# michaelnny/muzero

Measured on AMD Instinct MI355X. Metric: self-play MCTS sims/sec (env-steps/sec = value / sims_per_move), higher is better.
Workload: dtype f32

## Files before the change

### include/mzlearner.h

```cpp
#ifndef MZLEARNER_H
#define MZLEARNER_H

#include <stdint.h>

#ifdef __cplusplus
extern "C" {
#endif

#define MZL_OK 0
#define MZL_E_INVALID (-1)
#define MZL_E_HIP (-2)
#define MZL_E_STATE (-3)

#define MZL_NET_MLP 0
#define MZL_NET_BOARD 1
#define MZL_NET_ATARI 2

typedef struct {
    int32_t in_dim;
    int32_t num_actions;
    int32_t num_planes;
    int32_t hidden_dim;
    int32_t value_support_size;
    int32_t reward_support_size;
// ... 15 lines not shown
    const int64_t* d_index;
    const float* d_weights;
    float* d_loss;
    float* d_priorities;
    int32_t batch;
    int32_t state_is_int8;
    int32_t action_bytes;
} mzl_batch;

typedef struct mz_learner mz_learner;

const char* mzl_last_error(void);


int mzl_create(const mzl_config* cfg, int device_id, mz_learner** out);
int mzl_destroy(mz_learner* h);

int64_t mzl_num_params(const mz_learner* h);
int64_t mzl_grad_floats(const mz_learner* h);
int32_t mzl_num_tensors(const mz_learner* h);
int mzl_tensor_info(const mz_learner* h, int32_t i, const char** name, int64_t* offset, int32_t* rows, int32_t* cols);
int32_t mzl_num_buffers(const mz_learner* h);
int64_t mzl_num_running(const mz_learner* h);
int mzl_buffer_info(const mz_learner* h, int32_t i, const char** name, int64_t* offset, int32_t* count);
int mzl_bind_buffers(mz_learner* h, float* d_running, int64_t* d_num_batches);

int mzl_bind(mz_learner* h, float* d_params, float* d_grads, float* d_exp_avg, float* d_exp_avg_sq);
int mzl_commit(mz_learner* h, void* stream);

int mzl_grad(mz_learner* h, const mzl_batch* batch, void* stream);
// ... 26 lines not shown
```

### muzero_amd/csrc/learner.hip

```cpp
#include <hip/hip_runtime.h>

#include <cmath>
#include <cstdio>
#include <cstdlib>
#include <cstring>
#include <string>
#include <vector>

#include "../../include/mzlearner.h"
#include "mz_learn.h"
#include "mz_learn_conv_host.h"

using namespace mzl;

static thread_local std::string g_err;
static int fail(int code, const std::string& msg) {
    g_err = msg;
    return code;
}
void mzl_internal_set_error(const std::string& msg) { g_err = msg; }
#define HIPCHK(expr)                                                                                                                     \
    do {                                                                                                                                 \
        hipError_t _e = (expr);                                                                                                          \
        if (_e != hipSuccess)                                                                                                            \
// ... 21 lines not shown
    int lds_heads = 0;
    std::vector<void*> allocs;
    DwJob* d_jobs = nullptr;
    DwBig* d_big = nullptr;
    std::vector<DwBig> big;
    std::vector<DwJob> jobs;
    int jobs_tiles = -1;
    float* d_sq = nullptr;
    int sq_blocks = 0;
    int num_cus = 256;
    const void* checked_ptr[9] = {};
    int fast_max_tiles = 16, stage_fast_max_tiles = 256;
    int chain_min_tiles = 96, chain_max_tiles = 1 << 30;
    float *params = nullptr, *grads = nullptr, *m = nullptr, *v = nullptr;
    bool committed = false;
    int back_parts = 1;
    bool fast = false;
};

static int tiles16(int x) { return (x + 15) / 16; }

extern "C" const char* mzl_last_error(void) { return g_err.c_str(); }

template <typename T>
static hipError_t dalloc(mz_learner* h, T** p, size_t count) {
    void* q = nullptr;
    hipError_t e = hipMalloc(&q, count * sizeof(T) + 256);
    if (e != hipSuccess) return e;
    e = hipMemset(q, 0, count * sizeof(T) + 256);
    h->allocs.push_back(q);
// ... 208 lines not shown
        h->fast = n.p_t <= 4 * LW && n.in_t <= 6 && n.h_t + n.a_t <= 6 && n.h_t <= 4 && n.a_t <= 2 && n.sv_t <= 2 && n.sr_t <= 2 && n.h_t * 64 <= LT &&
                  ks_ok(n.h_t, n.p_t) && ks_ok(n.a_t, n.p_t) && ks_ok(n.sv_t, n.p_t) && ks_ok(n.sr_t, n.p_t) && !getenv("MZL_GENERIC");
    }
    {
        const bool ok = h->fast && n.p_t % DX_PARTS == 0 && n.p_t / DX_PARTS <= LW && n.h_t <= 4 && LW % n.h_t == 0 && (n.p_t / DX_PARTS) % (LW / n.h_t) == 0 &&
                        (n.p_t / DX_PARTS) / (LW / n.h_t) <= 4 && n.h_t * 64 <= LT && !getenv("MZL_NO_SLICE");
        h->back_parts = ok ? DX_PARTS : 1;
    }
    build_jobs(h);
    build_big_jobs(h);
    if (dalloc(h, &h->d_jobs, h->jobs.size()) != hipSuccess || dalloc(h, &h->d_big, h->big.size()) != hipSuccess) return cleanup(fail(MZL_E_HIP, "hipMalloc failed (jobs)"));
    hipError_t e = hipSuccess;
    const void* stage_kernels[] = {(const void*)&k_learn_repr<true>,   (const void*)&k_learn_repr<false>, (const void*)&k_learn_unroll<true>,
                                   (const void*)&k_learn_unroll<false>, (const void*)&k_learn_back<true>,  (const void*)&k_learn_back<false>,
                                   (const void*)&k_learn_back_sliced<true>, (const void*)&k_learn_fwd_sliced<true>,
                                   (const void*)&k_learn_unroll<false, 3>, (const void*)&k_learn_dyn_chain, (const void*)&k_learn_dyn_back_chain};
    for (const void* f : stage_kernels)
        if (e == hipSuccess) e = hipFuncSetAttribute(f, hipFuncAttributeMaxDynamicSharedMemorySize, 160 * 1024);
    if (e == hipSuccess) e = hipFuncSetAttribute(reinterpret_cast<const void*>(&k_learn_dw), hipFuncAttributeMaxDynamicSharedMemorySize, LW * 8 * 256 * 4);
    if (e != hipSuccess) return cleanup(fail(MZL_E_HIP, std::string("hipFuncSetAttribute: ") + hipGetErrorString(e)));
    e = hipDeviceSynchronize();
    if (e != hipSuccess) return cleanup(fail(MZL_E_HIP, std::string("hipDeviceSynchronize: ") + hipGetErrorString(e)));
    *out = h;
    return MZL_OK;
}

extern "C" int mzl_destroy(mz_learner* h) {
    if (!h) return MZL_OK;
    (void)hipSetDevice(h->device);
    (void)hipDeviceSynchronize();
    if (h->conv) mzlc_destroy(h->conv);
    for (void* p : h->allocs) (void)hipFree(p);
    delete h;
    return MZL_OK;
}

extern "C" void* mzl_debug_stamps(const mz_learner* h) { return h ? h->sv.stamps : nullptr; }

extern "C" int64_t mzl_num_params(const mz_learner* h) { return !h ? 0 : (h->conv ? mzlc_num_params(h->conv) : h->P.total); }
extern "C" int64_t mzl_grad_floats(const mz_learner* h) {
    return !h ? 0 : (h->conv ? mzlc_num_params(h->conv) : (int64_t)h->P.total * h->cfg.grad_slices);
}
extern "C" int32_t mzl_num_tensors(const mz_learner* h) { return !h ? 0 : (h->conv ? mzlc_num_tensors(h->conv) : 2 * NLAYER); }
extern "C" int32_t mzl_num_buffers(const mz_learner* h) { return (h && h->conv) ? mzlc_num_buffers(h->conv) : 0; }
extern "C" int64_t mzl_num_running(const mz_learner* h) { return (h && h->conv) ? mzlc_num_running(h->conv) : 0; }
extern "C" int mzl_buffer_info(const mz_learner* h, int32_t i, const char** name, int64_t* offset, int32_t* count) {
    if (!h || !h->conv || mzlc_buffer_info(h->conv, i, name, offset, count) != MZL_OK) return fail(MZL_E_INVALID, "buffer index out of range");
// ... 10 lines not shown
    return MZL_OK;
}

extern "C" int mzl_tensor_info(const mz_learner* h, int32_t i, const char** name, int64_t* offset, int32_t* rows, int32_t* cols) {
    if (h && h->conv) {
        if (mzlc_tensor_info(h->conv, i, name, offset, rows, cols) != MZL_OK) return fail(MZL_E_INVALID, "tensor index out of range");
        return MZL_OK;
    }
    if (!h || i < 0 || i >= 2 * NLAYER) return fail(MZL_E_INVALID, "tensor index out of range");
    const LTensor& t = h->P.t[i];
    if (name) *name = h->names[i].c_str();
    if (offset) *offset = t.off;
    if (rows) *rows = t.n;
    if (cols) *cols = t.k;
    return MZL_OK;
}

extern "C" int mzl_bind(mz_learner* h, float* d_params, float* d_grads, float* d_exp_avg, float* d_exp_avg_sq) {
    if (!h || !d_params || !d_grads || !d_exp_avg || !d_exp_avg_sq) return fail(MZL_E_INVALID, "null argument to mzl_bind");
    if (h->conv) return mzlc_bind(h->conv, d_params, d_grads, d_exp_avg, d_exp_avg_sq);
    h->params = d_params; h->grads = d_grads; h->m = d_exp_avg; h->v = d_exp_avg_sq;
    h->committed = false;
    h->jobs_tiles = -1;
    return MZL_OK;
}

static int launch_adam(mz_learner* h, const AdamArgs& a, hipStream_t st) {
    int maxcnt = 0;
    for (int i = 0; i < 2 * NLAYER; i++) {
        const LTensor& t = h->P.t[i];
// ... 40 lines not shown
        static const char* names[9] = {"d_state", "d_action", "d_pi_prob", "d_value", "d_reward", "d_index", "d_weights", "d_loss", "d_priorities"};
        for (int i = 0; i < 9; i++) {
            if (ptrs[i] == h->checked_ptr[i]) continue;
            hipPointerAttribute_t at{};
            const hipError_t e = hipPointerGetAttributes(&at, ptrs[i]);
            if (e != hipSuccess || at.type != hipMemoryTypeDevice || at.device != h->device) {
                (void)hipGetLastError();
                return fail(MZL_E_INVALID, std::string(names[i]) + " is not memory of the learner's GPU (the batch is read where the replay lives: keep it in HBM)");
            }
            h->checked_ptr[i] = ptrs[i];
        }
    }
    if (b->action_bytes == 1 && h->cfg.num_actions > 128) return fail(MZL_E_INVALID, "num_actions > 128 needs int16 actions");
    HIPCHK(hipSetDevice(h->device));
    hipStream_t st = reinterpret_cast<hipStream_t>(stream);
    const LNet& n = h->net;
    LBatch bt{};
    bt.state = b->d_state; bt.action = b->d_action; bt.pi = b->d_pi_prob; bt.value = b->d_value; bt.reward = b->d_reward;
    bt.idx = b->d_index; bt.w = b->d_weights; bt.prio = b->d_priorities; bt.B = b->batch; bt.tiles = tiles16(b->batch);
    bt.state_i8 = b->state_is_int8; bt.action_bytes = b->action_bytes;
    const int tiles = bt.tiles, K = n.K;
    if (h->jobs_tiles != tiles) {
        std::vector<DwJob> jj = h->jobs;
        for (auto& j : jj) j.R *= tiles;
        std::vector<DwBig> bb = h->big;
        for (auto& j : bb) j.R *= tiles;
        HIPCHK(hipMemcpyAsync(h->d_jobs, jj.data(), jj.size() * sizeof(DwJob), hipMemcpyHostToDevice, st));
        HIPCHK(hipMemcpyAsync(h->d_big, bb.data(), bb.size() * sizeof(DwBig), hipMemcpyHostToDevice, st));
        HIPCHK(hipMemsetAsync(h->grads, 0, (size_t)h->P.total * h->cfg.grad_slices * sizeof(float), st));
        HIPCHK(hipStreamSynchronize(st));
        h->jobs_tiles = tiles;
    }
    const size_t lds = (size_t)h->lds_bytes;
    const int fast_max_tiles = h->fast_max_tiles;
    const int chain_max_tiles = h->stage_fast_max_tiles;
    const bool fast_heads = h->fast && tiles < fast_max_tiles;
    const bool fast_chain_base = h->fast && (fast_heads || tiles <= chain_max_tiles);
    const bool chain = h->fast && n.h_t * 64 <= LT && tiles >= h->chain_min_tiles && tiles <= h->chain_max_tiles;
    const int sliced_ok = (h->back_parts > 1 && tiles * h->back_parts <= 512) ? h->back_parts : 1;
    const bool fast_chain = fast_chain_base || chain;
    const int fparts = (!chain && fast_chain && sliced_ok > 1 && n.in_t <= WKG && n.h_t + n.a_t <= WKG) ? h->back_parts : 1;
    if (fast_chain) {
        if (fparts > 1) {
            for (int k = -1; k < K; k++) hipLaunchKernelGGL(k_learn_fwd_sliced<true>, dim3(tiles, fparts), dim3(LT), lds, st, n, h->sv, bt, h->o, k, fparts);
            hipLaunchKernelGGL(k_learn_fwd_sliced<true>, dim3(tiles, 1), dim3(LT), lds, st, n, h->sv, bt, h->o, K, fparts);
        } else if (chain) {
            if (fast_chain_base) hipLaunchKernelGGL(k_learn_repr<true>, dim3(tiles), dim3(LT), lds, st, n, h->sv, bt, h->o);
            else hipLaunchKernelGGL(k_learn_repr<false>, dim3(tiles), dim3(LT), lds, st, n, h->sv, bt, h->o);
            hipLaunchKernelGGL(k_learn_dyn_chain, dim3(tiles < h->num_cus ? tiles : h->num_cus), dim3(LT), lds, st, n, h->sv, bt, h->o);
        } else {
            hipLaunchKernelGGL(k_learn_repr<true>, dim3(tiles), dim3(LT), lds, st, n, h->sv, bt, h->o);
            for (int k = 0; k < K; k++) hipLaunchKernelGGL(k_learn_unroll<true>, dim3(tiles), dim3(LT), lds, st, n, h->sv, bt, h->o, k, 0);
        }
    } else {
        hipLaunchKernelGGL(k_learn_repr<false>, dim3(tiles), dim3(LT), lds, st, n, h->sv, bt, h->o);
        for (int k = 0; k < K; k++) hipLaunchKernelGGL(k_learn_unroll<false>, dim3(tiles), dim3(LT), lds, st, n, h->sv, bt, h->o, k, 0);
    }
    if (fast_heads) {
        hipLaunchKernelGGL(k_learn_unroll<true>, dim3(tiles, 3, K), dim3(LT), lds, st, n, h->sv, bt, h->o, 0, 1);
    } else {
        static const bool heads3_on = !getenv("MZL_NO_HEADS3");
        const bool heads3 = heads3_on && n.p_t <= 4 * LW && n.a_t <= 2 && n.sv_t <= 2 && n.sr_t <= 2 && 3 * (h->lds_heads + 512) <= 160 * 1024;
        if (heads3) hipLaunchKernelGGL((k_learn_unroll<false, 3>), dim3(tiles, 3, K), dim3(LT), (size_t)h->lds_heads, st, n, h->sv, bt, h->o_heads, 0, 1);
        else hipLaunchKernelGGL(k_learn_unroll<false>, dim3(tiles, 3, K), dim3(LT), lds, st, n, h->sv, bt, h->o, 0, 1);
    }
    if (fast_chain) {
        LSave svb = h->sv;
        svb.dx_parts = chain ? 1 : sliced_ok;
        if (svb.dx_parts > 1) {
            for (int k = K - 1; k >= -1; k--) hipLaunchKernelGGL(k_learn_back_sliced<true>, dim3(tiles, svb.dx_parts), dim3(LT), lds, st, n, svb, bt, h->o, k);
        } else if (chain) {
            hipLaunchKernelGGL(k_learn_dyn_back_chain, dim3(tiles < h->num_cus ? tiles : h->num_cus), dim3(LT), lds, st, n, svb, bt, h->o);
            if (fast_chain_base) hipLaunchKernelGGL(k_learn_back<true>, dim3(tiles), dim3(LT), lds, st, n, svb, bt, h->o, -1);
            else hipLaunchKernelGGL(k_learn_back<false>, dim3(tiles), dim3(LT), lds, st, n, svb, bt, h->o, -1);
        } else {
            for (int k = K - 1; k >= -1; k--) hipLaunchKernelGGL(k_learn_back<true>, dim3(tiles), dim3(LT), lds, st, n, svb, bt, h->o, k);
        }
    } else {
        for (int k = K - 1; k >= -1; k--) hipLaunchKernelGGL(k_learn_back<false>, dim3(tiles), dim3(LT), lds, st, n, h->sv, bt, h->o, k);
    }
    const int n_loss = 3 * K * tiles;
// ... 40 lines not shown
```

### muzero_amd/csrc/mz_learn.h

```cpp
#pragma once
#include <type_traits>

#include "mz_device.h"

namespace mzl {

typedef float f32x4 __attribute__((ext_vector_type(4)));

constexpr int LW = 8;
constexpr int LT = LW * 64;
constexpr int TILE = 16;
constexpr int RPS = LT / TILE;
constexpr int DX_PARTS = 4;

__device__ __forceinline__ int pk(int k, int e) { return (((k >> 4) * 64 + ((k >> 2) & 3) * 16 + e) << 2) + (k & 3); }

enum { REP0 = 0, REP1, DYN0, DYN1, REW0, REW1, POL0, POL1, VAL0, VAL1, NLAYER };

struct LLayer {
    const float* wp;
    const float* wtp;
    const float* b;
    int n, k;
    int nt, kg;
// ... 259 lines not shown
__device__ __forceinline__ f32x4 g_get_T(const float* blocks, int t, int lane) {
    const float4 v = reinterpret_cast<const float4*>(blocks)[t * 64 + lane];
    return f32x4{v.x, v.y, v.z, v.w};
}
__device__ __forceinline__ void save_T_from_pk(const float* lds, int nt, float* blocks, int tid) {
    for (int u = tid; u < nt * 64; u += LT) {
        const int t = u >> 6, lane = u & 63, f = lane & 15, sq = lane >> 4;
        const float* p = lds + (((t * 64 + (f >> 2) * 16 + 4 * sq) << 2) + (f & 3));
        reinterpret_cast<float4*>(blocks)[u] = make_float4(p[0], p[4], p[8], p[12]);
    }
}
__device__ __forceinline__ void copy_f4(float* dst, const float* src, int nfloat4, int tid) {
    for (int i = tid; i < nfloat4; i += LT) reinterpret_cast<float4*>(dst)[i] = reinterpret_cast<const float4*>(src)[i];
}

__device__ __forceinline__ float half_sum(float v) {
    v = mz::butterfly16(v);
    return v + __shfl_xor(v, 16, 64);
}
__device__ __forceinline__ float half_max(float v) {
    v = mz::butterfly16_max(v);
    const float o = __shfl_xor(v, 16, 64);
    return o > v ? o : v;
}
__device__ __forceinline__ float half_min(float v) {
    v = mz::butterfly16_min(v);
    const float o = __shfl_xor(v, 16, 64);
    return o < v ? o : v;
}

// ... 180 lines not shown
        const f32x4 r = {fmaxf(a[0], 0.0f), fmaxf(a[1], 0.0f), fmaxf(a[2], 0.0f), fmaxf(a[3], 0.0f)};
        g_put_T(h1b, t, lane, r);
        lds_put_T(lds + o.H1, t, lane, r);
    }, NoPf{});
    __syncthreads();
    ks_mma<F>(w2, net.L[REP1].wp, net.L[REP1].b, net.h_t, net.p_t, lds + o.H1, lds + o.RED, wave, lane,
           [&](int t, f32x4 a) { lds_put_T(lds + o.HN, t, lane, a); }, NoPf{});
    __syncthreads();
    normalize_fwd(lds + o.HN, lds + o.HS, net.H, net.h_t, tid);
    __syncthreads();
    const size_t cb = blk(0, tiles, tile, net.h_t);
    copy_f4(sv.uc + cb, lds + o.HN, net.h_t * 64, tid);
    copy_f4(sv.hc + cb, lds + o.HS, net.h_t * 64, tid);
}

template <bool F, int OCC = 1>
__global__ __launch_bounds__(LT, OCC * LW / 4) void k_learn_unroll(LNet net, LSave sv, LBatch bt, LLds o, int k0, int role0) {
    extern __shared__ __align__(16) float lds[];
    const int tid = threadIdx.x, lane = tid & 63, wave = __builtin_amdgcn_readfirstlane(tid >> 6), tile = blockIdx.x, tiles = bt.tiles;
    const int role = role0 + (int)blockIdx.y, k = k0 + (int)blockIdx.z + ((role == 3 && gridDim.y > 1) ? 1 : 0);
    const int K = net.K, hf = net.h_t * 64;
    const int e = tid >> 5, j = tid & 31, s = tile * TILE + e;
    WideW w1;
    KsW w2;
    if (OCC != 3 && role == 0) {
        if (k >= K) return;
        MZL_STAMP(0);
        const float* hsrc = sv.hc + blk(k, tiles, tile, net.h_t);
        const float4 xv = chain_ld(hsrc, hf, tid);
        const int act = sv.actc[(k * tiles + tile) * TILE + e];
        wide_load<6, true, F>(w1, net.L[DYN0].wp, net.L[DYN0].b, net.p_t, net.h_t + net.a_t, wave, lane);
        chain_st<F>(lds + o.X, hsrc, xv, hf, tid);
        for (int a = j; a < net.a_t * 16; a += 32) lds[o.X + pk(net.h_t * 16 + a, e)] = a == act ? 1.0f : 0.0f;
        __syncthreads();
        MZL_STAMP(1);
// ... 17 lines not shown
        const size_t cb = blk(k + 1, tiles, tile, net.h_t);
        copy_f4(sv.uc + cb, lds + o.HN, hf, tid);
        copy_f4(sv.hc + cb, lds + o.HS, hf, tid);
        MZL_STAMP(5);
        return;
    }
    const int step = role == 3 ? k - 1 : k;
    if (step < 0 || step >= K) return;
    const int l0 = role == 1 ? POL0 : (role == 2 ? VAL0 : REW0), l1 = l0 + 1;
    const int S = role == 1 ? net.A : (role == 2 ? net.Sv : net.Sr), s_t = role == 1 ? net.a_t : (role == 2 ? net.sv_t : net.sr_t);
    const int sb = 16 * role;
    MZL_STAMP(sb + 0);
    const bool valid = s < bt.B;
    const int row = sample_row(bt, s);
    const float* xsrc = (role == 3 ? sv.uc : sv.hc) + blk(k, tiles, tile, net.h_t);
    const float4 xv = chain_ld(xsrc, hf, tid);
    wide_load<4, true, F>(w1, net.L[l0].wp, net.L[l0].b, net.p_t, net.h_t, wave, lane);
    const float wl = bt.w[s < bt.B ? s : bt.B - 1], w = valid ? wl : 0.0f;
    const float tgt = (role == 2 ? bt.value : bt.reward)[(size_t)row * K + step];
    const float* pi_row = bt.pi + ((size_t)row * K + step) * net.A;
    const float pi_first = pi_row[j < net.A ? j : 0];
    float* h1_all = role == 1 ? sv.h1_pol : (role == 2 ? sv.h1_val : sv.h1_rew);
    float* dz0_all = role == 1 ? sv.dz_pol0 : (role == 2 ? sv.dz_val0 : sv.dz_rew0);
    float* dz1_all = role == 1 ? sv.dz_pol1 : (role == 2 ? sv.dz_val1 : sv.dz_rew1);
    float* dx_all = role == 1 ? sv.dxp : (role == 2 ? sv.dxv : sv.dxr);
    chain_st<F>(lds + o.X, xsrc, xv, hf, tid);
    __syncthreads();
    MZL_STAMP(sb + 1);
    ks_load<true, F>(w2, net.L[l1].wp, net.L[l1].b, s_t, net.p_t, wave, lane);
    MZL_STAMP(sb + 8);
    if (role == 3) save_T_from_pk(lds + o.X, net.h_t, sv.u_in + blk(step, tiles, tile, net.h_t), tid);
// ... 46 lines not shown
            const int jj = (t - wave) / LW;
            h = jj == 0 ? h1k[0] : (jj == 1 ? h1k[1] : (jj == 2 ? h1k[2] : h1k[3]));
        } else {
            h = g_get_T(h1b, t, lane);
        }
        const f32x4 r = {h[0] > 0.0f ? a[0] : 0.0f, h[1] > 0.0f ? a[1] : 0.0f, h[2] > 0.0f ? a[2] : 0.0f, h[3] > 0.0f ? a[3] : 0.0f};
        g_put_T(dzb, t, lane, r);
        lds_put_T(lds + o.DZ, t, lane, r);
    }, NoPf{});
    __syncthreads();
    MZL_STAMP(sb + 5);
    ks_mma<F>(w2, net.L[l0].wtp, nullptr, net.h_t, net.p_t, lds + o.DZ, lds + o.RED, wave, lane,
           [&](int t, f32x4 a) { lds_put_T(lds + o.G, t, lane, a); }, NoPf{});
    __syncthreads();
    MZL_STAMP(sb + 6);
    copy_f4(dx_all + blk(step, tiles, tile, net.h_t), lds + o.G, hf, tid);
    MZL_STAMP(sb + 7);
}

template <bool F>
__global__ __launch_bounds__(LT) void k_learn_fwd_sliced(LNet net, LSave sv, LBatch bt, LLds o, int k, int np) {
    extern __shared__ __align__(16) float lds[];
    const int tid = threadIdx.x, lane = tid & 63, wave = __builtin_amdgcn_readfirstlane(tid >> 6), tile = blockIdx.x, tiles = bt.tiles;
    const int part = blockIdx.y, K = net.K, hf = net.h_t * 64;
    const int e = tid >> 5, jr = tid & 31, smp = tile * TILE + e;
    const int l0 = k < 0 ? REP0 : DYN0, l1 = l0 + 1, kg1 = k < 0 ? net.in_t : net.h_t + net.a_t;
    const int tb = part * net.p_t / np, te = (part + 1) * net.p_t / np;
    const int ci = tid < hf ? tid : hf - 1;
    float4 us = make_float4(0.0f, 0.0f, 0.0f, 0.0f);
    int act = -1;
    const int kk = k < 0 ? 0 : k;
    {
        const float* ub = sv.up + blk(kk, tiles, tile, net.h_t) * DX_PARTS;
#pragma unroll
        for (int pp = 0; pp < DX_PARTS; pp++) {
            const float4 v = reinterpret_cast<const float4*>(ub + (size_t)(pp < np ? pp : 0) * net.h_t * 256)[ci];
            const float m = pp < np ? 1.0f : 0.0f;
            us = make_float4(us.x + m * v.x, us.y + m * v.y, us.z + m * v.z, us.w + m * v.w);
        }
        const float* bsrc = (k <= 0 ? net.L[REP1].b : net.L[DYN1].b) + (ci >> 6) * 16 + ((ci >> 4) & 3) * 4;
        const float4 bv = *reinterpret_cast<const float4*>(bsrc);
        us = make_float4(us.x + bv.x, us.y + bv.y, us.z + bv.z, us.w + bv.w);
        act = sv.actc[((kk < K ? kk : K - 1) * tiles + tile) * TILE + e];
    }
    const int row = sample_row(bt, smp);
    const int t = tb + wave < te ? tb + wave : te - 1;
    const bool t_ok = tb + wave < te && k < K;
    const float4* W1 = reinterpret_cast<const float4*>(net.L[l0].wp) + lane;
    float4 w1[WKG];
#pragma unroll
    for (int d = 0; d < WKG; d++) w1[d] = ldg4(W1 + ((size_t)t * kg1 + (d < kg1 ? d : kg1 - 1)) * 64);
    const float b1 = net.L[l0].b[t * 16 + (lane & 15)];
    const int kparts = LW / net.h_t, ot = wave % net.h_t, kp = wave / net.h_t;
    const int nb = (te - tb) / kparts, g0 = tb + kp * nb;
    const float4* W2 = reinterpret_cast<const float4*>(net.L[l1].wp) + ((size_t)ot * net.p_t) * 64 + lane;
    float4 w2[4];
#pragma unroll
    for (int d = 0; d < 4; d++) w2[d] = ldg4(W2 + (size_t)(g0 + (d < nb ? d : nb - 1)) * 64);
    if (k < 0) {
        const bool valid = smp < bt.B;
        for (int f = jr; f < net.in_t * 16; f += 32) {
            float v = 0.0f;
            if (valid && f < net.in_dim)
                v = bt.state_i8 ? (float)reinterpret_cast<const int8_t*>(bt.state)[(size_t)row * net.in_dim + f]
                                : reinterpret_cast<const float*>(bt.state)[(size_t)row * net.in_dim + f];
            lds[o.X + pk(f, e)] = v;
        }
        if (part == 0 && jr < K) sv.actc[(jr * tiles + tile) * TILE + e] = valid ? sample_action(bt, row, K, jr) : -1;
        __syncthreads();
        if (part == 0) save_T_from_pk(lds + o.X, net.in_t, sv.in_rep + blk(0, tiles, tile, net.in_t), tid);
    } else {
        if (tid < hf) reinterpret_cast<float4*>(lds + o.HN)[tid] = us;
        __syncthreads();
        normalize_fwd(lds + o.HN, lds + o.X, net.H, net.h_t, tid);
        for (int a = jr; a < net.a_t * 16; a += 32) lds[o.X + pk(net.h_t * 16 + a, e)] = a == act ? 1.0f : 0.0f;
        __syncthreads();
        if (part == 0) {
            const size_t cb = blk(k, tiles, tile, net.h_t);
            copy_f4(sv.uc + cb, lds + o.HN, hf, tid);
            copy_f4(sv.hc + cb, lds + o.X, hf, tid);
            if (k < K) save_T_from_pk(lds + o.X, net.h_t + net.a_t, sv.x + blk(k, tiles, tile, net.h_t + net.a_t), tid);
        }
        if (k >= K) return;
    }
    float* h1b = (k < 0 ? sv.h1_rep : sv.h1_dyn) + blk(kk, tiles, tile, net.p_t);
    if (t_ok) {
        const float4* X4 = reinterpret_cast<const float4*>(lds + o.X) + lane;
        f32x4 a = {b1, b1, b1, b1};
#pragma unroll
        for (int d = 0; d < WKG; d++)
            if (d < kg1) a = mfma4(X4[d * 64], w1[d], a);
        const f32x4 r = {fmaxf(a[0], 0.0f), fmaxf(a[1], 0.0f), fmaxf(a[2], 0.0f), fmaxf(a[3], 0.0f)};
        g_put_T(h1b, t, lane, r);
        lds_put_T(lds + o.H1, t, lane, r);
    }
// ... 4 lines not shown
#pragma unroll
        for (int d = 0; d < 4; d++)
            if (d < nb) a = mfma4(X4[(g0 + d) * 64], w2[d], a);
        reinterpret_cast<float4*>(lds + o.RED)[(kp * net.h_t + ot) * 64 + lane] = make_float4(a[0], a[1], a[2], a[3]);
    }
    __syncthreads();
    if (wave < net.h_t) {
        f32x4 sacc = {0.0f, 0.0f, 0.0f, 0.0f};
        for (int q = 0; q < kparts; q++) {
            const float4 v = reinterpret_cast<const float4*>(lds + o.RED)[(q * net.h_t + wave) * 64 + lane];
            sacc = sacc + f32x4{v.x, v.y, v.z, v.w};
        }
        lds_put_T(lds + o.G, wave, lane, sacc);
    }
    __syncthreads();
    copy_f4(sv.up + blk(k + 1, tiles, tile, net.h_t) * DX_PARTS + (size_t)part * net.h_t * 256, lds + o.G, hf, tid);
}

template <bool F>
__global__ __launch_bounds__(LT) void k_learn_back(LNet net, LSave sv, LBatch bt, LLds o, int k) {
    extern __shared__ __align__(16) float lds[];
    const int tid = threadIdx.x, lane = tid & 63, wave = __builtin_amdgcn_readfirstlane(tid >> 6), tile = blockIdx.x, tiles = bt.tiles;
    const int K = net.K, j = k + 1;
    const int hf = net.h_t * 64;
    const int l0 = k >= 0 ? DYN0 : REP0, l1 = l0 + 1;
    const int st = k >= 0 ? k : 0;
    const size_t cj = blk(j, tiles, tile, net.h_t);
    const int ci = tid < hf ? tid : hf - 1;
    const float4 z4 = make_float4(0.0f, 0.0f, 0.0f, 0.0f);
    const bool cons = j < K;
    const size_t cjc = cons ? cj : 0;
// ... 141 lines not shown
                const int jj = (t - wave) / LW;
                const f32x4 h = jj == 0 ? gk[0] : (jj == 1 ? gk[1] : (jj == 2 ? gk[2] : gk[3]));
                const f32x4 r = {h[0] > 0.0f ? a[0] : 0.0f, h[1] > 0.0f ? a[1] : 0.0f, h[2] > 0.0f ? a[2] : 0.0f, h[3] > 0.0f ? a[3] : 0.0f};
                g_put_T(dzb, t, lane, r);
                lds_put_T(lds + o.DZ, t, lane, r);
            }, NoPf{});
            __syncthreads();
            ks_mma<true>(w2, net.L[DYN0].wtp, nullptr, net.h_t, net.p_t, lds + o.DZ, lds + o.RED, wave, lane,
                         [&](int t, f32x4 a) { lds_put_T(lds + o.G, t, lane, a); }, NoPf{});
            __syncthreads();
        }
        copy_f4(sv.dxd + blk(0, tiles, tile, net.h_t) * DX_PARTS, lds + o.G, hf, tid);
    }
}

template <bool F>
__global__ __launch_bounds__(LT) void k_learn_back_sliced(LNet net, LSave sv, LBatch bt, LLds o, int k) {
    extern __shared__ __align__(16) float lds[];
    const int tid = threadIdx.x, lane = tid & 63, wave = __builtin_amdgcn_readfirstlane(tid >> 6), tile = blockIdx.x, tiles = bt.tiles;
    const int part = blockIdx.y, np = gridDim.y, K = net.K, j = k + 1, hf = net.h_t * 64;
    const int l0 = k >= 0 ? DYN0 : REP0, l1 = l0 + 1, st = k >= 0 ? k : 0;
    const int tb = part * net.p_t / np, te = (part + 1) * net.p_t / np;
    const size_t cj = blk(j, tiles, tile, net.h_t);
    const int ci = tid < hf ? tid : hf - 1;
    const bool cons = j < K;
    const size_t cjc = cons ? cj : 0;
    float4 ga = make_float4(0.0f, 0.0f, 0.0f, 0.0f);
#pragma unroll
    for (int pp = 0; pp < DX_PARTS; pp++) {
        const float4 v = reinterpret_cast<const float4*>(sv.dxd + (cjc * DX_PARTS) + (size_t)(pp < sv.dx_parts ? pp : 0) * net.h_t * 256)[ci];
        const float m = pp < sv.dx_parts ? 1.0f : 0.0f;
        ga = make_float4(ga.x + m * v.x, ga.y + m * v.y, ga.z + m * v.z, ga.w + m * v.w);
    }
    const float4 gb = reinterpret_cast<const float4*>(sv.dxp + cjc)[ci], gc = reinterpret_cast<const float4*>(sv.dxv + cjc)[ci];
    const float4 uu = reinterpret_cast<const float4*>(sv.uc + cj)[ci];
    const float4 rr = reinterpret_cast<const float4*>(sv.dxr + blk(st, tiles, tile, net.h_t))[ci];
    const int t = tb + wave < te ? tb + wave : te - 1;
    const bool t_ok = tb + wave < te;
    const float4* W2T = reinterpret_cast<const float4*>(net.L[l1].wtp) + lane;
    float4 w1[4];
#pragma unroll
    for (int d = 0; d < 4; d++) w1[d] = ldg4(W2T + ((size_t)t * net.h_t + (d < net.h_t ? d : net.h_t - 1)) * 64);
    const float* h1b = (k >= 0 ? sv.h1_dyn : sv.h1_rep) + blk(st, tiles, tile, net.p_t);
    const f32x4 gate = g_get_T(h1b, t, lane);
    const int kparts = LW / net.h_t, ot = wave % net.h_t, kp = wave / net.h_t;
    const int nb = (te - tb) / kparts, g0 = tb + kp * nb;
    const float4* W1T = reinterpret_cast<const float4*>(net.L[DYN0].wtp) + ((size_t)ot * net.p_t) * 64 + lane;
    float4 w2[4];
#pragma unroll
    for (int d = 0; d < 4; d++) w2[d] = ldg4(W1T + (size_t)(g0 + (d < nb ? d : nb - 1)) * 64);
    if (tid < hf) {
// ... 25 lines not shown
#pragma unroll
        for (int d = 0; d < 4; d++)
            if (d < nb) a = mfma4(X4[(g0 + d) * 64], w2[d], a);
        reinterpret_cast<float4*>(lds + o.RED)[(kp * net.h_t + ot) * 64 + lane] = make_float4(a[0], a[1], a[2], a[3]);
    }
    __syncthreads();
    if (wave < net.h_t) {
        f32x4 sacc = {0.0f, 0.0f, 0.0f, 0.0f};
        for (int q = 0; q < kparts; q++) {
            const float4 v = reinterpret_cast<const float4*>(lds + o.RED)[(q * net.h_t + wave) * 64 + lane];
            sacc = sacc + f32x4{v.x, v.y, v.z, v.w};
        }
        lds_put_T(lds + o.G, wave, lane, sacc);
    }
    __syncthreads();
    copy_f4(sv.dxd + blk(k, tiles, tile, net.h_t) * DX_PARTS + (size_t)part * net.h_t * 256, lds + o.G, hf, tid);
}

__device__ __forceinline__ void loss_finish(const float* __restrict__ lossp, int n, int B, float* __restrict__ loss_out, float* sc) {
    const int tid = threadIdx.x;
    float s0 = 0.0f, s1 = 0.0f, s2 = 0.0f, s3 = 0.0f;
    int i = tid;
    for (; i + 3 * LT < n; i += 4 * LT) {
        const float a = lossp[i], b = lossp[i + LT], c = lossp[i + 2 * LT], d = lossp[i + 3 * LT];
        s0 += a; s1 += b; s2 += c; s3 += d;
    }
    for (; i < n; i += LT) s0 += lossp[i];
    sc[tid] = (s0 + s1) + (s2 + s3);
    __syncthreads();
    for (int m = LT / 2; m > 0; m >>= 1) {
        if (tid < m) sc[tid] += sc[tid + m];
// ... 273 lines not shown
```

### muzero_amd/hip_learner.py

```python
import ctypes as C
import os
from typing import Optional, Sequence

import numpy as np
import torch

_HERE = os.path.dirname(os.path.abspath(__file__))
LIB_PATH = os.path.join(_HERE, 'lib', 'libmzlearner_hip.so')

ABI_SYMBOLS = ['mzl_last_error', 'mzl_create', 'mzl_destroy', 'mzl_num_params', 'mzl_grad_floats', 'mzl_num_tensors', 'mzl_tensor_info',
               'mzl_num_buffers', 'mzl_num_running', 'mzl_buffer_info', 'mzl_bind_buffers', 'mzl_bind', 'mzl_commit', 'mzl_grad', 'mzl_apply',
               'mzl_replay_scratch_doubles', 'mzl_replay_sample', 'mzl_replay_update_priorities', 'mzl_replay_set_error_counters']
NET_MLP, NET_BOARD, NET_ATARI = 0, 1, 2


class LearnerError(RuntimeError):
    pass


class MzlConfig(C.Structure):
    _fields_ = [('in_dim', C.c_int32), ('num_actions', C.c_int32), ('num_planes', C.c_int32), ('hidden_dim', C.c_int32),
                ('value_support_size', C.c_int32), ('reward_support_size', C.c_int32), ('unroll_steps', C.c_int32), ('max_batch', C.c_int32),
                ('grad_slices', C.c_int32), ('net_kind', C.c_int32), ('in_channels', C.c_int32), ('board_h', C.c_int32), ('board_w', C.c_int32),
                ('num_res_blocks', C.c_int32)]

# ... 12 lines not shown

_lib = None


def load_library():
    global _lib
    if _lib is not None:
        return _lib
    if not os.path.exists(LIB_PATH):
        raise LearnerError(f'{LIB_PATH} not found: build it with `python -m muzero_amd.build` (hipcc, gfx950). The HIP learner has no CPU fallback.')
    L = C.CDLL(LIB_PATH)
    vp, i32, i64 = C.c_void_p, C.c_int32, C.c_int64
    L.mzl_last_error.restype = C.c_char_p
    L.mzl_create.argtypes = [C.POINTER(MzlConfig), C.c_int, C.POINTER(vp)]
    L.mzl_destroy.argtypes = [vp]
    L.mzl_num_params.argtypes = [vp]
    L.mzl_num_params.restype = i64
    L.mzl_grad_floats.argtypes = [vp]
    L.mzl_grad_floats.restype = i64
    L.mzl_tensor_info.argtypes = [vp, i32, C.POINTER(C.c_char_p), C.POINTER(i64), C.POINTER(i32), C.POINTER(i32)]
    L.mzl_num_tensors.argtypes = [vp]
    L.mzl_num_tensors.restype = i32
    L.mzl_num_buffers.argtypes = [vp]
    L.mzl_num_buffers.restype = i32
    L.mzl_num_running.argtypes = [vp]
    L.mzl_num_running.restype = i64
    L.mzl_buffer_info.argtypes = [vp, i32, C.POINTER(C.c_char_p), C.POINTER(i64), C.POINTER(i32)]
    L.mzl_bind_buffers.argtypes = [vp, vp, vp]
    L.mzl_bind.argtypes = [vp, vp, vp, vp, vp]
    L.mzl_commit.argtypes = [vp, vp]
# ... 280 lines not shown
        return loss, prio

    def step_transitions(self, transitions, weights=None):
        def dev(x, dt):
            t = x if torch.is_tensor(x) else torch.from_numpy(np.ascontiguousarray(x))
            return t.to(self.device, dt).contiguous()

        st = transitions.state
        st_dt = torch.int8 if (torch.is_tensor(st) and st.dtype == torch.int8) or (not torch.is_tensor(st) and np.asarray(st).dtype == np.int8) else torch.float32
        B = int(st.shape[0])
        ring = dict(state=dev(st, st_dt).reshape(B, -1), action=dev(transitions.action, torch.int16 if self.A > 128 else torch.int8),
                    pi_prob=dev(transitions.pi_prob, torch.float32), value=dev(transitions.value, torch.float32), reward=dev(transitions.reward, torch.float32))
        w = None if weights is None else dev(weights, torch.float32)
        return self.step(ring, None, w, B)

    def close(self) -> None:
        if self._h:
            load_library().mzl_destroy(self._h)
            self._h = C.c_void_p()

    def __del__(self):
        try:
            self.close()
        except Exception:
            pass
```

Before: 292.5 million.

## Fuse small MLP learner step into one cooperative kernel with counter hand-offs

Adds a cooperative kernel k_learn_step_small. It runs the plane-sliced forward chain, the prediction heads and the sliced backward chain in a single launch, with workgroups handing off through per-tile global atomic counters and spin-waits. Data passed between stages uses agent-scope relaxed atomic loads and stores. The aim is to remove the per-unroll-step kernel launches and inter-kernel gaps of the learner. The cost is spin-wait overhead, a timeout and error path, and the need for all workgroups to be co-resident.

Result: no change. 293.2 million, median of 2 (+0.2%).

```diff
diff --git a/include/mzlearner.h b/include/mzlearner.h
--- a/include/mzlearner.h
+++ b/include/mzlearner.h
@@ -53,6 +53,7 @@
 
 
 int mzl_create(const mzl_config* cfg, int device_id, mz_learner** out);
+const char* mzl_describe(const mz_learner* h);
 int mzl_destroy(mz_learner* h);
 
 int64_t mzl_num_params(const mz_learner* h);
diff --git a/muzero_amd/csrc/learner.hip b/muzero_amd/csrc/learner.hip
--- a/muzero_amd/csrc/learner.hip
+++ b/muzero_amd/csrc/learner.hip
@@ -59,6 +59,11 @@
     int chain_min_tiles = 96, chain_max_tiles = 1 << 30;
     float *params = nullptr, *grads = nullptr, *m = nullptr, *v = nullptr;
     bool committed = false;
+    int fused_max_grid = 0;
+    int* d_sync = nullptr;
+    int* h_err = nullptr;
+    int sync_bank = 0, sync_cap_tiles = 16;
+    std::string last_path = "none yet";
     int back_parts = 1;
     bool fast = false;
 };
@@ -297,11 +302,26 @@
     const void* stage_kernels[] = {(const void*)&k_learn_repr<true>,   (const void*)&k_learn_repr<false>, (const void*)&k_learn_unroll<true>,
                                    (const void*)&k_learn_unroll<false>, (const void*)&k_learn_back<true>,  (const void*)&k_learn_back<false>,
                                    (const void*)&k_learn_back_sliced<true>, (const void*)&k_learn_fwd_sliced<true>,
-                                   (const void*)&k_learn_unroll<false, 3>, (const void*)&k_learn_dyn_chain, (const void*)&k_learn_dyn_back_chain};
+                                   (const void*)&k_learn_unroll<false, 3>, (const void*)&k_learn_dyn_chain, (const void*)&k_learn_dyn_back_chain,
+                                   (const void*)&k_learn_step_small};
     for (const void* f : stage_kernels)
         if (e == hipSuccess) e = hipFuncSetAttribute(f, hipFuncAttributeMaxDynamicSharedMemorySize, 160 * 1024);
     if (e == hipSuccess) e = hipFuncSetAttribute(reinterpret_cast<const void*>(&k_learn_dw), hipFuncAttributeMaxDynamicSharedMemorySize, LW * 8 * 256 * 4);
     if (e != hipSuccess) return cleanup(fail(MZL_E_HIP, std::string("hipFuncSetAttribute: ") + hipGetErrorString(e)));
+    {
+        const char* sw = getenv("MZ_LEARN_FUSED");
+        int coop = 0, nb = 0;
+        if (!(sw && atoi(sw) == 0) && h->back_parts > 1 && hipDeviceGetAttribute(&coop, hipDeviceAttributeCooperativeLaunch, device_id) == hipSuccess && coop &&
+            hipOccupancyMaxActiveBlocksPerMultiprocessor(&nb, reinterpret_cast<const void*>(&k_learn_step_small), LT, (size_t)h->lds_bytes) == hipSuccess && nb > 0) {
+            const size_t ints = (size_t)2 * xs_count(n.K, h->sync_cap_tiles) * XS;
+            void* he = nullptr;
+            if (dalloc(h, &h->d_sync, ints) != hipSuccess || hipHostMalloc(&he, 64) != hipSuccess) return cleanup(fail(MZL_E_HIP, "allocation failed (hand-off counters)"));
+            h->h_err = reinterpret_cast<int*>(he);
+            *h->h_err = 0;
+            h->fused_max_grid = h->num_cus;
+        }
+        (void)hipGetLastError();
+    }
     e = hipDeviceSynchronize();
     if (e != hipSuccess) return cleanup(fail(MZL_E_HIP, std::string("hipDeviceSynchronize: ") + hipGetErrorString(e)));
     *out = h;
@@ -314,6 +334,7 @@
     (void)hipDeviceSynchronize();
     if (h->conv) mzlc_destroy(h->conv);
     for (void* p : h->allocs) (void)hipFree(p);
+    if (h->h_err) (void)hipHostFree(h->h_err);
     delete h;
     return MZL_OK;
 }
@@ -354,6 +375,15 @@
     if (rows) *rows = t.n;
     if (cols) *cols = t.k;
     return MZL_OK;
+}
+
+static thread_local std::string g_describe;
+extern "C" const char* mzl_describe(const mz_learner* h) {
+    if (!h) return "";
+    if (h->conv) g_describe = "conv learner (learner_conv.hip)";
+    else g_describe = "mlp learner: " + h->last_path + " | MZ_LEARN_FUSED=" + std::to_string(h->fused_max_grid > 0 ? 1 : 0) +
+                      " hand_off_error=" + std::to_string(h->h_err ? *(volatile int*)h->h_err : 0);
+    return g_describe.c_str();
 }
 
 extern "C" int mzl_bind(mz_learner* h, float* d_params, float* d_grads, float* d_exp_avg, float* d_exp_avg_sq) {
@@ -424,6 +454,14 @@
     if (b->action_bytes == 1 && h->cfg.num_actions > 128) return fail(MZL_E_INVALID, "num_actions > 128 needs int16 actions");
     HIPCHK(hipSetDevice(h->device));
     hipStream_t st = reinterpret_cast<hipStream_t>(stream);
+    if (h->h_err && *(volatile int*)h->h_err) {
+        const int code = *(volatile int*)h->h_err;
+        HIPCHK(hipDeviceSynchronize());
+        HIPCHK(hipMemset(h->d_sync, 0, (size_t)2 * xs_count(h->net.K, h->sync_cap_tiles) * XS * sizeof(int)));
+        *h->h_err = 0;
+        h->sync_bank = 0;
+        return fail(MZL_E_HIP, "k_learn_step_small: a hand-off wait of an earlier step ran out (stage code " + std::to_string(code) + ")");
+    }
     const LNet& n = h->net;
     LBatch bt{};
     bt.state = b->d_state; bt.action = b->d_action; bt.pi = b->d_pi_prob; bt.value = b->d_value; bt.reward = b->d_reward;
@@ -450,7 +488,25 @@
     const int sliced_ok = (h->back_parts > 1 && tiles * h->back_parts <= 512) ? h->back_parts : 1;
     const bool fast_chain = fast_chain_base || chain;
     const int fparts = (!chain && fast_chain && sliced_ok > 1 && n.in_t <= WKG && n.h_t + n.a_t <= WKG) ? h->back_parts : 1;
-    if (fast_chain) {
+    const int fgrid = tiles * fparts + 3 * (K + 1) * tiles;
+    const bool fused = h->fused_max_grid > 0 && fparts > 1 && sliced_ok == fparts && fast_heads && tiles <= h->sync_cap_tiles && fgrid <= h->fused_max_grid;
+    if (fused) {
+        LSave svf = h->sv;
+        svf.dx_parts = fparts;
+        LNet nn = n;
+        LLds oo = h->o;
+        int np = fparts;
+        LStepSync sy{h->d_sync, h->h_err, h->sync_bank, h->sync_cap_tiles, xs_count(K, h->sync_cap_tiles)};
+        void* args[] = {&nn, &svf, &bt, &oo, &np, &sy};
+        HIPCHK(hipLaunchCooperativeKernel(reinterpret_cast<const void*>(&k_learn_step_small), dim3(fgrid), dim3(LT), args, (unsigned)lds, st));
+        h->sync_bank ^= 1;
+        h->last_path = "one launch: k_learn_step_small, " + std::to_string(fgrid) + " workgroups (" + std::to_string(tiles * fparts) + " chain + " +
+                       std::to_string(fgrid - tiles * fparts) + " heads)";
+    } else {
+        h->last_path = "multi-launch stages (" + std::string(fparts > 1 ? "plane-sliced chains" : (chain ? "persistent chains" : "per-tile stages")) + ")";
+    }
+    if (fused) {
+    } else if (fast_chain) {
         if (fparts > 1) {
             for (int k = -1; k < K; k++) hipLaunchKernelGGL(k_learn_fwd_sliced<true>, dim3(tiles, fparts), dim3(LT), lds, st, n, h->sv, bt, h->o, k, fparts);
             hipLaunchKernelGGL(k_learn_fwd_sliced<true>, dim3(tiles, 1), dim3(LT), lds, st, n, h->sv, bt, h->o, K, fparts);
@@ -466,7 +522,8 @@
         hipLaunchKernelGGL(k_learn_repr<false>, dim3(tiles), dim3(LT), lds, st, n, h->sv, bt, h->o);
         for (int k = 0; k < K; k++) hipLaunchKernelGGL(k_learn_unroll<false>, dim3(tiles), dim3(LT), lds, st, n, h->sv, bt, h->o, k, 0);
     }
-    if (fast_heads) {
+    if (fused) {
+    } else if (fast_heads) {
         hipLaunchKernelGGL(k_learn_unroll<true>, dim3(tiles, 3, K), dim3(LT), lds, st, n, h->sv, bt, h->o, 0, 1);
     } else {
         static const bool heads3_on = !getenv("MZL_NO_HEADS3");
@@ -474,7 +531,8 @@
         if (heads3) hipLaunchKernelGGL((k_learn_unroll<false, 3>), dim3(tiles, 3, K), dim3(LT), (size_t)h->lds_heads, st, n, h->sv, bt, h->o_heads, 0, 1);
         else hipLaunchKernelGGL(k_learn_unroll<false>, dim3(tiles, 3, K), dim3(LT), lds, st, n, h->sv, bt, h->o, 0, 1);
     }
-    if (fast_chain) {
+    if (fused) {
+    } else if (fast_chain) {
         LSave svb = h->sv;
         svb.dx_parts = chain ? 1 : sliced_ok;
         if (svb.dx_parts > 1) {
diff --git a/muzero_amd/csrc/mz_learn.h b/muzero_amd/csrc/mz_learn.h
--- a/muzero_amd/csrc/mz_learn.h
+++ b/muzero_amd/csrc/mz_learn.h
@@ -297,6 +297,45 @@
     for (int i = tid; i < nfloat4; i += LT) reinterpret_cast<float4*>(dst)[i] = reinterpret_cast<const float4*>(src)[i];
 }
 
+template <bool X>
+__device__ __forceinline__ float4 xld4(const float* base, int i) {
+    if constexpr (!X) {
+        return reinterpret_cast<const float4*>(base)[i];
+    } else {
+        typedef const __attribute__((address_space(1))) float* gp_t;
+        gp_t p = (gp_t)(base + 4 * (size_t)i);
+        const float a = __hip_atomic_load(p, __ATOMIC_RELAXED, __HIP_MEMORY_SCOPE_AGENT), b = __hip_atomic_load(p + 1, __ATOMIC_RELAXED, __HIP_MEMORY_SCOPE_AGENT),
+                    c = __hip_atomic_load(p + 2, __ATOMIC_RELAXED, __HIP_MEMORY_SCOPE_AGENT), d = __hip_atomic_load(p + 3, __ATOMIC_RELAXED, __HIP_MEMORY_SCOPE_AGENT);
+        return make_float4(a, b, c, d);
+    }
+}
+template <bool X>
+__device__ __forceinline__ void copy_f4x(float* dst, const float* src, int nfloat4, int tid) {
+    if constexpr (!X) {
+        copy_f4(dst, src, nfloat4, tid);
+    } else {
+        typedef __attribute__((address_space(1))) float* gp_t;
+        for (int i = tid; i < nfloat4; i += LT) {
+            const float4 v = reinterpret_cast<const float4*>(src)[i];
+            gp_t p = (gp_t)(dst + 4 * (size_t)i);
+            __hip_atomic_store(p, v.x, __ATOMIC_RELAXED, __HIP_MEMORY_SCOPE_AGENT);
+            __hip_atomic_store(p + 1, v.y, __ATOMIC_RELAXED, __HIP_MEMORY_SCOPE_AGENT);
+            __hip_atomic_store(p + 2, v.z, __ATOMIC_RELAXED, __HIP_MEMORY_SCOPE_AGENT);
+            __hip_atomic_store(p + 3, v.w, __ATOMIC_RELAXED, __HIP_MEMORY_SCOPE_AGENT);
+        }
+    }
+}
+template <bool X>
+__device__ __forceinline__ int xldi(const int* p) {
+    if constexpr (!X) return *p;
+    else return __hip_atomic_load((const __attribute__((address_space(1))) int*)p, __ATOMIC_RELAXED, __HIP_MEMORY_SCOPE_AGENT);
+}
+template <bool X>
+__device__ __forceinline__ void xsti(int* p, int v) {
+    if constexpr (!X) *p = v;
+    else __hip_atomic_store((__attribute__((address_space(1))) int*)p, v, __ATOMIC_RELAXED, __HIP_MEMORY_SCOPE_AGENT);
+}
+
 __device__ __forceinline__ float half_sum(float v) {
     v = mz::butterfly16(v);
     return v + __shfl_xor(v, 16, 64);
@@ -507,11 +546,9 @@
     copy_f4(sv.hc + cb, lds + o.HS, net.h_t * 64, tid);
 }
 
-template <bool F, int OCC = 1>
-__global__ __launch_bounds__(LT, OCC * LW / 4) void k_learn_unroll(LNet net, LSave sv, LBatch bt, LLds o, int k0, int role0) {
-    extern __shared__ __align__(16) float lds[];
-    const int tid = threadIdx.x, lane = tid & 63, wave = __builtin_amdgcn_readfirstlane(tid >> 6), tile = blockIdx.x, tiles = bt.tiles;
-    const int role = role0 + (int)blockIdx.y, k = k0 + (int)blockIdx.z + ((role == 3 && gridDim.y > 1) ? 1 : 0);
+template <bool F, int OCC, bool X>
+__device__ __forceinline__ void unroll_body(const LNet& net, const LSave& sv, const LBatch& bt, const LLds& o, int role, int k, int tile, float* lds) {
+    const int tid = threadIdx.x, lane = tid & 63, wave = __builtin_amdgcn_readfirstlane(tid >> 6), tiles = bt.tiles;
     const int K = net.K, hf = net.h_t * 64;
     const int e = tid >> 5, j = tid & 31, s = tile * TILE + e;
     WideW w1;
@@ -559,7 +596,7 @@
     const bool valid = s < bt.B;
     const int row = sample_row(bt, s);
     const float* xsrc = (role == 3 ? sv.uc : sv.hc) + blk(k, tiles, tile, net.h_t);
-    const float4 xv = chain_ld(xsrc, hf, tid);
+    const float4 xv = X ? xld4<X>(xsrc, tid < hf ? tid : hf - 1) : chain_ld(xsrc, hf, tid);
     wide_load<4, true, F>(w1, net.L[l0].wp, net.L[l0].b, net.p_t, net.h_t, wave, lane);
     const float wl = bt.w[s < bt.B ? s : bt.B - 1], w = valid ? wl : 0.0f;
     const float tgt = (role == 2 ? bt.value : bt.reward)[(size_t)row * K + step];
@@ -636,15 +673,20 @@
            [&](int t, f32x4 a) { lds_put_T(lds + o.G, t, lane, a); }, NoPf{});
     __syncthreads();
     MZL_STAMP(sb + 6);
-    copy_f4(dx_all + blk(step, tiles, tile, net.h_t), lds + o.G, hf, tid);
+    copy_f4x<X>(dx_all + blk(step, tiles, tile, net.h_t), lds + o.G, hf, tid);
     MZL_STAMP(sb + 7);
 }
-
-template <bool F>
-__global__ __launch_bounds__(LT) void k_learn_fwd_sliced(LNet net, LSave sv, LBatch bt, LLds o, int k, int np) {
+template <bool F, int OCC = 1>
+__global__ __launch_bounds__(LT, OCC * LW / 4) void k_learn_unroll(LNet net, LSave sv, LBatch bt, LLds o, int k0, int role0) {
     extern __shared__ __align__(16) float lds[];
-    const int tid = threadIdx.x, lane = tid & 63, wave = __builtin_amdgcn_readfirstlane(tid >> 6), tile = blockIdx.x, tiles = bt.tiles;
-    const int part = blockIdx.y, K = net.K, hf = net.h_t * 64;
+    const int role = role0 + (int)blockIdx.y, k = k0 + (int)blockIdx.z + ((role == 3 && gridDim.y > 1) ? 1 : 0);
+    unroll_body<F, OCC, false>(net, sv, bt, o, role, k, blockIdx.x, lds);
+}
+
+template <bool F, bool X>
+__device__ __forceinline__ void fwd_sliced_body(const LNet& net, const LSave& sv, const LBatch& bt, const LLds& o, int k, int np, int tile, int part, float* lds) {
+    const int tid = threadIdx.x, lane = tid & 63, wave = __builtin_amdgcn_readfirstlane(tid >> 6), tiles = bt.tiles;
+    const int K = net.K, hf = net.h_t * 64;
     const int e = tid >> 5, jr = tid & 31, smp = tile * TILE + e;
     const int l0 = k < 0 ? REP0 : DYN0, l1 = l0 + 1, kg1 = k < 0 ? net.in_t : net.h_t + net.a_t;
     const int tb = part * net.p_t / np, te = (part + 1) * net.p_t / np;
@@ -656,14 +698,14 @@
         const float* ub = sv.up + blk(kk, tiles, tile, net.h_t) * DX_PARTS;
 #pragma unroll
         for (int pp = 0; pp < DX_PARTS; pp++) {
-            const float4 v = reinterpret_cast<const float4*>(ub + (size_t)(pp < np ? pp : 0) * net.h_t * 256)[ci];
+            const float4 v = xld4<X>(ub + (size_t)(pp < np ? pp : 0) * net.h_t * 256, ci);
             const float m = pp < np ? 1.0f : 0.0f;
             us = make_float4(us.x + m * v.x, us.y + m * v.y, us.z + m * v.z, us.w + m * v.w);
         }
         const float* bsrc = (k <= 0 ? net.L[REP1].b : net.L[DYN1].b) + (ci >> 6) * 16 + ((ci >> 4) & 3) * 4;
         const float4 bv = *reinterpret_cast<const float4*>(bsrc);
         us = make_float4(us.x + bv.x, us.y + bv.y, us.z + bv.z, us.w + bv.w);
-        act = sv.actc[((kk < K ? kk : K - 1) * tiles + tile) * TILE + e];
+        act = xldi<X>(sv.actc + ((kk < K ? kk : K - 1) * tiles + tile) * TILE + e);
     }
     const int row = sample_row(bt, smp);
     const int t = tb + wave < te ? tb + wave : te - 1;
@@ -688,7 +730,7 @@
                                 : reinterpret_cast<const float*>(bt.state)[(size_t)row * net.in_dim + f];
             lds[o.X + pk(f, e)] = v;
         }
-        if (part == 0 && jr < K) sv.actc[(jr * tiles + tile) * TILE + e] = valid ? sample_action(bt, row, K, jr) : -1;
+        if (part == 0 && jr < K) xsti<X>(sv.actc + (jr * tiles + tile) * TILE + e, valid ? sample_action(bt, row, K, jr) : -1);
         __syncthreads();
         if (part == 0) save_T_from_pk(lds + o.X, net.in_t, sv.in_rep + blk(0, tiles, tile, net.in_t), tid);
     } else {
@@ -699,8 +741,8 @@
         __syncthreads();
         if (part == 0) {
             const size_t cb = blk(k, tiles, tile, net.h_t);
-            copy_f4(sv.uc + cb, lds + o.HN, hf, tid);
-            copy_f4(sv.hc + cb, lds + o.X, hf, tid);
+            copy_f4x<X>(sv.uc + cb, lds + o.HN, hf, tid);
+            copy_f4x<X>(sv.hc + cb, lds + o.X, hf, tid);
             if (k < K) save_T_from_pk(lds + o.X, net.h_t + net.a_t, sv.x + blk(k, tiles, tile, net.h_t + net.a_t), tid);
         }
         if (k >= K) return;
@@ -735,7 +777,12 @@
         lds_put_T(lds + o.G, wave, lane, sacc);
     }
     __syncthreads();
-    copy_f4(sv.up + blk(k + 1, tiles, tile, net.h_t) * DX_PARTS + (size_t)part * net.h_t * 256, lds + o.G, hf, tid);
+    copy_f4x<X>(sv.up + blk(k + 1, tiles, tile, net.h_t) * DX_PARTS + (size_t)part * net.h_t * 256, lds + o.G, hf, tid);
+}
+template <bool F>
+__global__ __launch_bounds__(LT) void k_learn_fwd_sliced(LNet net, LSave sv, LBatch bt, LLds o, int k, int np) {
+    extern __shared__ __align__(16) float lds[];
+    fwd_sliced_body<F, false>(net, sv, bt, o, k, np, blockIdx.x, blockIdx.y, lds);
 }
 
 template <bool F>
@@ -907,11 +954,10 @@
     }
 }
 
-template <bool F>
-__global__ __launch_bounds__(LT) void k_learn_back_sliced(LNet net, LSave sv, LBatch bt, LLds o, int k) {
-    extern __shared__ __align__(16) float lds[];
-    const int tid = threadIdx.x, lane = tid & 63, wave = __builtin_amdgcn_readfirstlane(tid >> 6), tile = blockIdx.x, tiles = bt.tiles;
-    const int part = blockIdx.y, np = gridDim.y, K = net.K, j = k + 1, hf = net.h_t * 64;
+template <bool F, bool X>
+__device__ __forceinline__ void back_sliced_body(const LNet& net, const LSave& sv, const LBatch& bt, const LLds& o, int k, int np, int tile, int part, float* lds) {
+    const int tid = threadIdx.x, lane = tid & 63, wave = __builtin_amdgcn_readfirstlane(tid >> 6), tiles = bt.tiles;
+    const int K = net.K, j = k + 1, hf = net.h_t * 64;
     const int l0 = k >= 0 ? DYN0 : REP0, l1 = l0 + 1, st = k >= 0 ? k : 0;
     const int tb = part * net.p_t / np, te = (part + 1) * net.p_t / np;
     const size_t cj = blk(j, tiles, tile, net.h_t);
@@ -921,13 +967,13 @@
     float4 ga = make_float4(0.0f, 0.0f, 0.0f, 0.0f);
 #pragma unroll
     for (int pp = 0; pp < DX_PARTS; pp++) {
-        const float4 v = reinterpret_cast<const float4*>(sv.dxd + (cjc * DX_PARTS) + (size_t)(pp < sv.dx_parts ? pp : 0) * net.h_t * 256)[ci];
+        const float4 v = xld4<X>(sv.dxd + (cjc * DX_PARTS) + (size_t)(pp < sv.dx_parts ? pp : 0) * net.h_t * 256, ci);
         const float m = pp < sv.dx_parts ? 1.0f : 0.0f;
         ga = make_float4(ga.x + m * v.x, ga.y + m * v.y, ga.z + m * v.z, ga.w + m * v.w);
     }
-    const float4 gb = reinterpret_cast<const float4*>(sv.dxp + cjc)[ci], gc = reinterpret_cast<const float4*>(sv.dxv + cjc)[ci];
-    const float4 uu = reinterpret_cast<const float4*>(sv.uc + cj)[ci];
-    const float4 rr = reinterpret_cast<const float4*>(sv.dxr + blk(st, tiles, tile, net.h_t))[ci];
+    const float4 gb = xld4<X>(sv.dxp + cjc, ci), gc = xld4<X>(sv.dxv + cjc, ci);
+    const float4 uu = xld4<X>(sv.uc + cj, ci);
+    const float4 rr = xld4<X>(sv.dxr + blk(st, tiles, tile, net.h_t), ci);
     const int t = tb + wave < te ? tb + wave : te - 1;
     const bool t_ok = tb + wave < te;
     const float4* W2T = reinterpret_cast<const float4*>(net.L[l1].wtp) + lane;
@@ -983,7 +1029,82 @@
         lds_put_T(lds + o.G, wave, lane, sacc);
     }
     __syncthreads();
-    copy_f4(sv.dxd + blk(k, tiles, tile, net.h_t) * DX_PARTS + (size_t)part * net.h_t * 256, lds + o.G, hf, tid);
+    copy_f4x<X>(sv.dxd + blk(k, tiles, tile, net.h_t) * DX_PARTS + (size_t)part * net.h_t * 256, lds + o.G, hf, tid);
+}
+template <bool F>
+__global__ __launch_bounds__(LT) void k_learn_back_sliced(LNet net, LSave sv, LBatch bt, LLds o, int k) {
+    extern __shared__ __align__(16) float lds[];
+    back_sliced_body<F, false>(net, sv, bt, o, k, gridDim.y, blockIdx.x, blockIdx.y, lds);
+}
+
+constexpr int XS = 32;
+struct LStepSync {
+    int* ctr;
+    int* err;
+    int bank, cap_tiles, bank_counters;
+};
+__host__ __device__ inline int xs_count(int K, int cap_tiles) { return (3 * K + 4) * cap_tiles; }
+__device__ __forceinline__ void xsignal(int* ctr, int inc) {
+    asm volatile("s_waitcnt vmcnt(0)" ::: "memory");
+    __syncthreads();
+    if (threadIdx.x == 0) __hip_atomic_fetch_add(ctr, inc, __ATOMIC_RELAXED, __HIP_MEMORY_SCOPE_AGENT);
+}
+__device__ __forceinline__ bool xwait(const int* ctr, int lo, int* err, int code, int* flag) {
+    __syncthreads();
+    if (threadIdx.x == 0) {
+        typedef const __attribute__((address_space(1))) int* gp_t;
+        int ok = 1, n = 0;
+        long long t0 = 0;
+        while (__hip_atomic_load((gp_t)ctr, __ATOMIC_RELAXED, __HIP_MEMORY_SCOPE_AGENT) < lo) {
+            __builtin_amdgcn_s_sleep(2);
+            if ((++n & 255) == 0) {
+                const long long t = (long long)wall_clock64();
+                if (t0 == 0) t0 = t;
+                if (t - t0 > 200000000LL) { ok = 0; break; }
+            }
+        }
+        if (!ok) *(volatile int*)err = code;
+        *flag = ok;
+    }
+    __syncthreads();
+    const bool ok = *flag != 0;
+    return ok;
+}
+__global__ __launch_bounds__(LT) void k_learn_step_small(LNet net, LSave sv, LBatch bt, LLds o, int np, LStepSync sy) {
+    extern __shared__ __align__(16) float lds[];
+    const int tiles = bt.tiles, K = net.K, nchain = tiles * np, wg = blockIdx.x, ct = sy.cap_tiles;
+    int* flag = reinterpret_cast<int*>(lds + o.MISC + 32);
+    int* F = sy.ctr + (size_t)sy.bank * sy.bank_counters * XS;
+    int* B = F + (size_t)(K + 2) * ct * XS;
+    int* HD = B + (size_t)(K + 1) * ct * XS;
+    if (wg == gridDim.x - 1) {
+        int* other = sy.ctr + (size_t)(1 - sy.bank) * sy.bank_counters * XS;
+        for (int i = threadIdx.x; i < sy.bank_counters; i += LT)
+            __hip_atomic_store((__attribute__((address_space(1))) int*)(other + (size_t)i * XS), 0, __ATOMIC_RELAXED, __HIP_MEMORY_SCOPE_AGENT);
+    }
+    const int all = 16 + np - 1;
+    if (wg < nchain) {
+        const int tile = wg / np, part = wg % np;
+        for (int k = -1; k <= K; k++) {
+            if (k == K && part != 0) break;
+            if (k >= 0 && !xwait(F + (size_t)(k * ct + tile) * XS, all, sy.err, 100 + k, flag)) return;
+            fwd_sliced_body<true, true>(net, sv, bt, o, k, np, tile, part, lds);
+            xsignal(F + (size_t)((k + 1) * ct + tile) * XS, part == 0 ? 16 : 1);
+        }
+        for (int k = K - 1; k >= -1; k--) {
+            const int z = k + 1, nh = (z < K ? 2 : 0) + (z > 0 ? 1 : 0);
+            if (!xwait(HD + (size_t)(z * ct + tile) * XS, nh, sy.err, 200 + z, flag)) return;
+            if (z < K && !xwait(B + (size_t)(z * ct + tile) * XS, np, sy.err, 300 + z, flag)) return;
+            back_sliced_body<true, true>(net, sv, bt, o, k, np, tile, part, lds);
+            if (k >= 0) xsignal(B + (size_t)(k * ct + tile) * XS, 1);
+        }
+        return;
+    }
+    const int idx = wg - nchain, tile = idx % tiles, zr = idx / tiles, role = zr % 3 + 1, z = zr / 3;
+    if (z > K || (role < 3 && z == K) || (role == 3 && z == 0)) return;
+    if (!xwait(F + (size_t)((z + 1) * ct + tile) * XS, 16, sy.err, 400 + z, flag)) return;
+    unroll_body<true, 1, true>(net, sv, bt, o, role, z, tile, lds);
+    xsignal(HD + (size_t)(z * ct + tile) * XS, 1);
 }
 
 __device__ __forceinline__ void loss_finish(const float* __restrict__ lossp, int n, int B, float* __restrict__ loss_out, float* sc) {
diff --git a/muzero_amd/hip_learner.py b/muzero_amd/hip_learner.py
--- a/muzero_amd/hip_learner.py
+++ b/muzero_amd/hip_learner.py
@@ -8,7 +8,7 @@
 _HERE = os.path.dirname(os.path.abspath(__file__))
 LIB_PATH = os.path.join(_HERE, 'lib', 'libmzlearner_hip.so')
 
-ABI_SYMBOLS = ['mzl_last_error', 'mzl_create', 'mzl_destroy', 'mzl_num_params', 'mzl_grad_floats', 'mzl_num_tensors', 'mzl_tensor_info',
+ABI_SYMBOLS = ['mzl_last_error', 'mzl_create', 'mzl_destroy', 'mzl_describe', 'mzl_num_params', 'mzl_grad_floats', 'mzl_num_tensors', 'mzl_tensor_info',
                'mzl_num_buffers', 'mzl_num_running', 'mzl_buffer_info', 'mzl_bind_buffers', 'mzl_bind', 'mzl_commit', 'mzl_grad', 'mzl_apply',
                'mzl_replay_scratch_doubles', 'mzl_replay_sample', 'mzl_replay_update_priorities', 'mzl_replay_set_error_counters']
 NET_MLP, NET_BOARD, NET_ATARI = 0, 1, 2
@@ -51,6 +51,8 @@
     L.mzl_last_error.restype = C.c_char_p
     L.mzl_create.argtypes = [C.POINTER(MzlConfig), C.c_int, C.POINTER(vp)]
     L.mzl_destroy.argtypes = [vp]
+    L.mzl_describe.argtypes = [vp]
+    L.mzl_describe.restype = C.c_char_p
     L.mzl_num_params.argtypes = [vp]
     L.mzl_num_params.restype = i64
     L.mzl_grad_floats.argtypes = [vp]
@@ -361,6 +363,9 @@
         w = None if weights is None else dev(weights, torch.float32)
         return self.step(ring, None, w, B)
 
+    def describe(self) -> str:
+        return load_library().mzl_describe(self._h).decode()
+
     def close(self) -> None:
         if self._h:
             load_library().mzl_destroy(self._h)
```
